# kai422/DAS3R

Measured on AMD Instinct MI355X. Metric: render fwd+bwd Msplats/s at 1080p, higher is better.
Workload: dtype f32; 1 GPU; 1M random splats, 1920x1080, SH degree 3, forward+backward (BASELINE.json configs[3], constant P); splats_per_gpu=1000000, splats_per_gpu_final=1000000, init_steps=30, sh_degree=3, num_rendered=2614506, api=GaussianRasterizer.forward + autograd backward (drop-in surface), parallelism=1 independent scenes, one per GPU

## Files before the change

### das3r_amd/csrc/api.hip

```cpp
#include <stdarg.h>
#include <string.h>

#include <vector>

#include "host_state.h"
#include "preprocess_choice.h"
#include <algorithm>

namespace das3r {

static thread_local char g_err[512] = "";

void set_error(const char *fmt, ...) {
    va_list ap;
    va_start(ap, fmt);
    vsnprintf(g_err, sizeof(g_err), fmt, ap);
    va_end(ap);
}

struct ProfRec {
    const char *name;
    hipEvent_t start, stop;
};
static bool g_prof_on = false;
// ... 163 lines not shown
}

using namespace das3r;

extern "C" int das3r_abi_version(void) { return DAS3R_ABI_VERSION; }
extern "C" void das3r_reload_switches(void) { load_switches(); }
extern "C" void das3r_debug_inject_fault(uint32_t bits) {
    g_inject_fault = (int)bits;
    load_switches();
}
extern "C" void das3r_debug_mutate(uint32_t what) {
    g_mutate = (int)what;
    load_switches();
}
extern "C" const char *das3r_last_error(void) { return g_err; }
extern "C" int das3r_split_colour_switch(void) { return switches().split_colour; }
extern "C" int das3r_split_colour_rule(int32_t has_sh, int32_t sh_degree, int32_t P, int32_t binning_path, int32_t no_backward, int32_t forced) {
    return split_colour_rule(has_sh != 0, sh_degree, P, binning_path, no_backward != 0, forced) ? 1 : 0;
}

namespace {
struct PolicyOnState {
    Verdict v;
    Resume r;
    das3r_path_policy_state *s;
    explicit PolicyOnState(das3r_path_policy_state *state) : s(state) { policy_state_from(*s, &v, &r); }
    ~PolicyOnState() { policy_state_to(v, r, s); }
    PolicyInputs inputs(const das3r_path_policy_inputs *in) {
        return PolicyInputs{in->P, in->W, in->H, in->ntiles, in->tbits, in->tile_passes, in->too_long, in->want_bits, in->forced, in->onesweep != 0,
                            in->capacity_hint, in->capacity_exact != 0, &r};
    }
};
ForwardPlan plan_of(const das3r_path_policy_plan *p) {
    return ForwardPlan{p->local != 0, p->seg != 0, p->seg_bits, p->seg_passes, p->speculate != 0, p->cap, p->decide_fine != 0, p->gen};
}
}
extern "C" void das3r_debug_path_policy_fresh(das3r_path_policy_state *state, uint32_t gen) { policy_state_to(Verdict::fresh(gen), Resume(), state); }
extern "C" void das3r_debug_path_policy_plan(das3r_path_policy_state *state, const das3r_path_policy_inputs *in, das3r_path_policy_plan *out) {
    PolicyOnState on(state);
    const ForwardPlan p = plan_forward(on.v, on.inputs(in));
    *out = das3r_path_policy_plan{p.local, p.seg, p.seg_bits, p.seg_passes, p.speculate, p.decide_fine, p.gen, p.cap};
}
extern "C" int das3r_debug_path_policy_count(das3r_path_policy_state *state, const das3r_path_policy_inputs *in, const das3r_path_policy_plan *plan, int64_t I) {
    PolicyOnState on(state);
    return learn_count(on.v, I, on.inputs(in), plan_of(plan)) ? 1 : 0;
}
extern "C" int das3r_debug_path_policy_skew(das3r_path_policy_state *state, uint32_t longest, uint32_t crowd16, int64_t cap, int32_t ntiles) {
    PolicyOnState on(state);
    return learn_skew(on.v, longest, crowd16, cap, ntiles) ? 1 : 0;
}
extern "C" uint32_t das3r_debug_path_policy_hint(const das3r_path_policy_state *state) {
    Verdict v;
    Resume r;
    policy_state_from(*state, &v, &r);
    return backward_hint(v, (uint32_t)BUCKET);
}
extern "C" void das3r_debug_path_policy_forget(das3r_path_policy_state *state) {
    PolicyOnState on(state);
    forget(on.v);
}
extern "C" void das3r_debug_path_policy_resume(das3r_path_policy_state *state, uint32_t fine, uint32_t forwards) {
    PolicyOnState on(state);
    resume(on.v, on.r, fine != 0u, forwards);
}
extern "C" int das3r_debug_seg_dbits(int32_t tbits, int32_t passes) { return seg_dbits((int)tbits, (int)passes); }

extern "C" void das3r_debug_parse_switches(const char *const *names, const char *const *values, int32_t n, int32_t experiments, das3r_switches *out) {
    auto lookup = [&](const char *name) -> const char * {
        for (int32_t i = 0; i < n; i++)
            if (strcmp(names[i], name) == 0) return values[i];
        return nullptr;
    };
    switches_to(parse_switches(lookup, experiments != 0), out);
}
// ... 415 lines not shown
```

### das3r_amd/csrc/common.h

```cpp
#pragma once
#include <hip/hip_runtime.h>
#include <stdint.h>
#include <stdio.h>

#include "../../include/das3r_raster.h"
#include "kernel_choice.h"
#include "path_policy.h"
#include "pretransform_math.h"

#define TILE_X 16
#define TILE_Y 16
#define TILE_PIX 256
#define WAVE 64
#define NEAR_PLANE 0.001f

namespace das3r {

void set_error(const char *fmt, ...);

const Switches &switches();

#define HIP_TRY(expr)                                                                          \
    do {                                                                                       \
        hipError_t _e = (expr);                                                                \
// ... 112 lines not shown
constexpr uint32_t SHJAC_SAVED_FLAG = 4u;
constexpr uint32_t NO_BACKWARD_IN_FLAG = 8u;
constexpr uint32_t ANTIALIAS_FLAG = 16u;
struct Layout {
    das3r_raster_layout pub;
    size_t g_keyA, g_keyB, g_valA, g_valB, g_hist, g_totals, g_blocksums, g_count, g_off_by_gid, g_rect;
    size_t b_keyA, b_keyB, b_valA, b_valB, b_hist, b_totals, b_gid_of, b_slot;
    size_t b_e2;
    size_t b_ckpt;
    size_t d_ckpt, d_recs, d_dpix, d_bg, d_dz, d_bytes;
    size_t g_ghist, g_ticket, g_status, g_scan_status, g_ctrl_bytes;
    int64_t capacity;
    size_t b_ghist, b_ticket, b_status, b_ctrl_bytes;
    int tiles_x, tiles_y, ntiles, tbits, tile_passes;
    int chunksP, chunksI;
    int dbits, kbits, kshift;
    int part_passes;
    size_t g_dhist;
    size_t g_shjac;
    const uint32_t *dhist_ptr;
    size_t i_order;
};
static inline int seg_dbits(const Layout &L, int passes) { return seg_dbits(L.tbits, passes); }

struct LocalBin {
    float4 *ckpt;
    uint32_t *point_list, *slot_list;
    uint32_t *keys;
    uint32_t *host_flag;
    uint32_t flag_value;
    uint32_t last_g, cap;
    bool prefer_regions;
    const uint32_t *tile_order;
};
void compute_layout(int P, int64_t I, int W, int H, Layout *L, bool shjac = false);

struct EmitArgs {
    unsigned long long *status;
    uint32_t tag;
    uint32_t *ghist;
    uint32_t *err;
    uint32_t *tile_keys, *gids, *off_by_gid;
    uint32_t cap;
    int tbits;
    uint32_t *count;
    uint32_t *count_out;
};
constexpr int EMIT_SLOT_WORDS = 64 + 4 * 256;
constexpr int EMIT_STATUS_GRANULES = 1024;

constexpr int COLOUR_WGS_PER_CU = 4;
struct SideStream {
    hipStream_t stream;
    hipEvent_t fork, join;
    int colour_blocks;
};
int launch_preprocess(const das3r_raster_args *a, const das3r_raster_in *in, int32_t *radii, char *geom, char *img, char *binning_ctrl,
                      size_t binning_ctrl_bytes, const Layout &L, unsigned long long *arrive, uint32_t *host_out, uint32_t tag,
                      hipStream_t s, const EmitArgs *emit, uint32_t *dhist, uint32_t *dhist_next, bool aa ,
                      const SideStream *side = nullptr);
int launch_sh_colour(const das3r_raster_args *a, const das3r_raster_in *in, char *geom, const Layout &L, const SideStream *side);
int launch_mark_visible(int P, const float *means3D, const float *viewmatrix, uint8_t *present, hipStream_t s);
int launch_depth_sort(int P, char *geom, const Layout &L, int part, char *binning_ctrl, size_t binning_ctrl_bytes, bool debug, hipStream_t s);
int launch_scan(int P, char *geom, const Layout &L, uint32_t *host_out, uint32_t tag, bool debug, hipStream_t s, bool index_order = false);
int launch_scan_emit(int P, int64_t cap, const int32_t *radii, char *geom, char *binning, const Layout &L, uint32_t *host_out, uint32_t tag,
                     bool debug, hipStream_t s, bool index_order = false);
// ... 12 lines not shown
        x = PreXform{p->xyz, p->rot, p->scaling, p->opacity_raw, p->conf_flat, p->mask_index, p->R, p->t, p->Lq};
    }
    return x;
}
int launch_render_forward_regions(const das3r_raster_args *a, float *out_color, char *geom, char *binning, char *img, const Layout &L, const LocalBin &lb,
                                  hipStream_t s, float *out_invdepth, float4 *dckpt);
int launch_tile_lpt(char *img, const Layout &L, uint32_t cap, bool debug, hipStream_t s);
int launch_list_skew(const char *img, const char *binning, const char *geom, const Layout &L, uint32_t cap, uint32_t last_g, uint32_t *mailbox_words, uint32_t tag,
                     bool debug, hipStream_t s);
int launch_render_forward_slices(const das3r_raster_args *a, float *out_color, char *geom, char *binning, char *img, const Layout &L, const LocalBin &lb,
                                 hipStream_t s);
int launch_render_forward_lanes(const das3r_raster_args *a, float *out_color, char *geom, char *binning, char *img, const Layout &L,
                                const LocalBin &lb, hipStream_t s, float *out_invdepth, float4 *dckpt);
int launch_render_forward_rows(const das3r_raster_args *a, float *out_color, char *geom, char *binning, char *img, const Layout &L,
                               const LocalBin &lb, hipStream_t s, float *out_invdepth, float4 *dckpt);
int launch_render_backward_mfma(const das3r_raster_args *a, const float *dL_dpix, char *geom, char *binning, char *img, const Layout &L,
                                float *partial, hipStream_t s);
size_t stream_scratch_bytes(int64_t capacity);
int launch_render_backward_stream(const das3r_raster_args *a, const float *dL_dpix, char *geom, char *binning, char *img, const Layout &L,
                                  float *scratch, hipStream_t s);
int launch_render_backward_scan(const das3r_raster_args *a, const float *dL_dpix, char *geom, char *binning, char *img, const Layout &L,
                                float *partial, const BwdChoice &c, hipStream_t s);
int launch_render_backward_blk(const das3r_raster_args *a, const float *dL_dpix, char *geom, char *binning, char *img, const Layout &L,
                               float *partial, const BwdChoice &c, hipStream_t s);
int launch_render_backward_regions(const das3r_raster_args *a, const float *dL_dpix, char *geom, char *binning, char *img, const Layout &L,
                               float *partial, const BwdChoice &c, hipStream_t s);
constexpr int LOCAL_MAX = 1024;
bool grid_is_resident(int nblocks);
bool use_onesweep();
bool use_tight_rect();
int launch_binning(int P, int64_t I, int W, int H, const int32_t *radii, char *geom, char *binning, char *img, const Layout &L,
                   bool fused_scan, uint32_t *host_late, uint32_t tag, bool debug, hipStream_t s, uint32_t **dead_keys = nullptr,
                   uint32_t *emit_slot = nullptr ,
                   uint32_t *seg_host_flag = nullptr, uint32_t seg_flag_value = 0 );
int launch_segment_sort(int64_t cap, const uint32_t *n_ptr, const uint32_t *keys_final, int fbits, uint32_t *point_list, uint32_t *slot_list,
                        const uint32_t *depth_key, uint32_t last_g, uint32_t *scratch_keys, uint32_t *host_flag, uint32_t flag_value, bool debug,
                        hipStream_t s, int dbits, uint2 *ranges, const uint32_t *err, uint32_t *host_late, uint32_t tag, uint32_t inject);
int launch_render_forward(const das3r_raster_args *a, const float *colors_precomp, float *out_color, char *geom, char *binning,
                          char *img, const Layout &L, const LocalBin &lb, hipStream_t s, float *out_invdepth ,
                          float4 *dckpt );
int launch_depth_pass_inputs(int P, int npix, const char *geom, const Layout &L, char *binning, const float *dL_dinvdepth, hipStream_t s, bool debug);
int launch_depth_fold(int P, const char *geom, const Layout &L, float *partial, const float *partial_depth, float *dz, hipStream_t s, bool debug);
size_t focal_workspace_bytes(int P);
int launch_focal_grad(const das3r_raster_args *a, const das3r_raster_in *in, const char *geom, const Layout &L, const float *partial, bool quad_rows,
                      bool aa , float *sums , float *per_splat , float *workspace, hipStream_t s);
static inline const uint8_t *quad_rows_exist(const float *partial, const Layout &L, bool quad_rows) {
    const size_t cap_rows = L.capacity > 0 ? (size_t)L.capacity : 1;
    return quad_rows ? reinterpret_cast<const uint8_t *>(partial) + align_up(cap_rows * 4 * 12 * sizeof(float)) : nullptr;
}
int launch_render_backward(const das3r_raster_args *a, const float *dL_dpix, char *geom, char *binning, char *img, const Layout &L,
                           float *partial, hipStream_t s, bool *quad_rows, int64_t num_rendered, uint32_t fwd_flags );
int launch_render_aux_forward(int P, int W, int H, int C, const float *feat, float *out, const char *geom, const char *binning, const char *img,
                              const Layout &L, int64_t num_rendered, bool debug, hipStream_t s);
int launch_render_aux_adjoint(int P, int W, int H, int C, const float *dL_dout, float *dL_dfeat, int accumulate, float *partial, const char *geom,
                              const char *binning, const char *img, const Layout &L, int64_t num_rendered, bool debug, hipStream_t s);
int launch_aux_gather(int P, int C, const float *partial, float *dL_dfeat, const char *geom, const Layout &L, bool debug, hipStream_t s);
int launch_render_aux_backward(int P, int W, int H, int C, const float *feat, const float *dL_dout, const float *dL_dalpha, float *partial,
                               float *partial_f, const char *geom, const char *binning, const char *img, const Layout &L, bool debug, hipStream_t s);
int launch_count_live_pairs(const das3r_raster_args *a, char *geom, char *binning, char *img, const Layout &L, unsigned long long *out, hipStream_t s);
int launch_preprocess_backward(const das3r_raster_args *a, const das3r_raster_in *in, char *geom, char *binning, const Layout &L,
                               const das3r_raster_grads *g, const float *partial, hipStream_t s, bool quad_rows, const float *dz ,
                               bool aa );

#ifdef __HIPCC__
__device__ __forceinline__ int lane_id() { return __lane_id(); }

template <int CTRL, int ROW_MASK>
// ... 29 lines not shown
```

### das3r_amd/csrc/forward.hip

```cpp
#include <string.h>

#include <algorithm>
#include <vector>

#include "host_state.h"

namespace das3r {

constexpr int SPLIT_MIN_P = 1 << 18;
bool split_colour_rule(bool has_sh, int sh_degree, int P, int binning_path, bool no_backward, int forced) {
    if (!has_sh || sh_degree < 1 || binning_path != 1 || forced < 0 || P <= 0) return false;
    if (forced > 0) return true;
    return sh_degree >= 2 && P >= SPLIT_MIN_P && !no_backward;
}

struct PerStream {
    int dev;
    hipStream_t caller;
    SideStream side = {nullptr, nullptr, nullptr, 0};
    uint32_t *dhist = nullptr;
    uint32_t turn = 0;
};
struct PerStreams {
    std::vector<PerStream> all;
// ... 332 lines not shown

int ForwardCall::look_at_lists(LocalBin *lb) {
    int r;
    const int P = a->P;
    const int64_t cap = L.capacity;
    const bool by_shape = cap > 0 && quad_lanes(switches(), L.ntiles, L.capacity, false);
    if (plan.decide_fine && by_shape) {
        const uint32_t tag = next_tag(mb);
        if ((r = launch_list_skew(saved->img, saved->binning, saved->geom, L, (uint32_t)cap, (uint32_t)(P - 1), mb->dev + MB_LONGEST, tag, a->debug != 0, s))) return r;
        if ((r = mailbox_wait(mb, MB_SKEW_TAG, tag, s))) return r;
        const uint32_t longest = mb->host[MB_LONGEST], crowd16 = mb->host[MB_CROWD16];
        const int64_t mean = skew_mean(T->verdict, cap, L.ntiles);
        const bool now_fine = learn_skew(T->verdict, longest, crowd16, cap, L.ntiles);
        if (switches().verbose) fprintf(stderr, "[das3r] tile lists: longest %lld, mean %lld, %.1f of 64 consecutive entries in one quadrant -> %s kernels\n", (long long)longest,
                                        (long long)mean, crowd16 / 16.0, now_fine ? "2x2-region" : "block");
    }
    const bool fine = prefers_regions(T->verdict);
    lb->prefer_regions = fine;
    lb->tile_order = nullptr;
    if (tile_lpt_wanted(switches(), L.ntiles, L.capacity, false, fine)) {
        if ((r = launch_tile_lpt(saved->img, L, (uint32_t)cap, a->debug != 0, s))) return r;
        lb->tile_order = (const uint32_t *)(saved->img + L.i_order);
    }
    if (fine && by_shape) saved->flags |= backward_hint(T->verdict, (uint32_t)BUCKET);
    return DAS3R_OK;
}

int ForwardCall::bin_and_render(bool local_order, bool ctrl_zeroed, uint32_t *count_out, uint32_t count_out_tag, uint32_t *emit_slot) {
    int r;
    const int P = a->P;
    const int64_t cap = L.capacity;
    const bool fused_scan = use_onesweep();
    const bool seg = L.dbits > 0;
    if (!emit_slot) {
        if (fused_scan) {
            if ((r = launch_binning_scan_emit(P, cap, out->radii, saved->geom, saved->binning, L, ctrl_zeroed, count_out, count_out_tag, a->debug != 0,
                                              s, local_order || seg))) return r;
        } else if ((r = launch_scan(P, saved->geom, L, nullptr, 0, a->debug != 0, s))) return r;
    }
    uint32_t *host_late = nullptr;
    if (cap > 0 && (r = claim_check_slot(&host_late))) return r;
    uint32_t *dead_keys = nullptr;
    if ((r = launch_binning(P, cap, a->image_width, a->image_height, out->radii, saved->geom, saved->binning, saved->img, L, fused_scan, host_late, late_tag,
                            a->debug != 0, s, &dead_keys, emit_slot, mb->dev + MB_TOO_LONG, plan.gen))) return r;
    if ((r = colour_launch())) return r;
    LocalBin lb = {(float4 *)(saved->binning + L.b_ckpt), nullptr, nullptr, nullptr, nullptr, plan.gen, (uint32_t)(P - 1), (uint32_t)cap};
    if ((r = look_at_lists(&lb))) return r;
    if (local_order && cap > 0) {
        lb.point_list = (uint32_t *)(saved->binning + L.pub.point_list);
        lb.slot_list = (uint32_t *)(saved->binning + L.b_slot);
        lb.keys = dead_keys;
        lb.host_flag = mb->dev + MB_TOO_LONG;
    }
    if ((r = colour_join())) return r;
    return launch_render_forward(a, in->colors_precomp, out->out_color, saved->geom, saved->binning, saved->img, L, lb, s, out->out_invdepth,
                                 depth ? (float4 *)(saved->binning + L.d_ckpt) : nullptr);
}

int ForwardCall::read_count(int64_t *I) {
    const int rc = mailbox_wait(mb, MB_COUNT_TAG, count_tag, s);
    if (rc) return rc;
    if (a->prefiltered && mb->host[MB_FILTERED] == count_tag) {
        set_error("Point is filtered although prefiltered is set. This shouldn't happen!");
        return DAS3R_ERR_INVALID_ARG;
    }
    *I = (int64_t)mb->host[MB_COUNT];
    if (*I > CAPACITY_MAX) { set_error("num_rendered %lld exceeds 2^31", (long long)*I); return DAS3R_ERR_OVERFLOW; }
    return DAS3R_OK;
}

int ForwardCall::flow_fused_emit(int64_t *I) {
    int rc;
    if (!T->emit_ring) HIP_TRY(hipMalloc((void **)&T->emit_ring, ARRIVE_SLOTS * EMIT_SLOT_BYTES));
    if (T->emit.wants_zeroing(count_tag)) {
        HIP_TRY(hipMemsetAsync(T->emit_ring, 0, ARRIVE_SLOTS * EMIT_SLOT_BYTES, s));
        T->emit.zeroed();
    }
    uint32_t *emit_slot = (uint32_t *)(T->emit_ring + (size_t)(count_tag % ARRIVE_SLOTS) * EMIT_SLOT_BYTES);
    const EmitArgs em = {(unsigned long long *)(emit_slot + EMIT_SLOT_WORDS), count_tag, emit_slot + 64, emit_slot,
                         (uint32_t *)(saved->binning + L.b_keyA), (uint32_t *)(saved->binning + L.b_gid_of),
                         (uint32_t *)(saved->geom + L.g_off_by_gid), (uint32_t)L.capacity, L.tbits, (uint32_t *)(saved->geom + L.g_count), mb->dev};
    T->emit.taken_by(count_tag);
    if ((rc = preprocess(2, &em))) return rc;
    if ((rc = bin_and_render(true, true, nullptr, 0, emit_slot))) return rc;
    T->emit.rearmed();
// ... 64 lines not shown
```

### das3r_amd/csrc/kernel_choice.h

```cpp
#pragma once
#include <stdint.h>
#include <stdlib.h>
#include <string.h>

#include <algorithm>

namespace das3r {

enum FwdKernel : int {
    FWD_AUTO = 0,
    FWD_QUAD = 1,
    FWD_ROWS = 2,
    FWD_LANES = 3,
    FWD_SLICES = 4,
    FWD_REGIONS = 5,
};
enum BwdKernel : int {
    BWD_AUTO = 0,
    BWD_DPP = 1,
    BWD_MFMA = 2,
    BWD_SCAN = 3,
    BWD_STREAM = 5,
    BWD_BLK = 6,
    BWD_REGIONS = 7,
// ... 53 lines not shown
    int ablate;
    int tickets;
    int bwd_pad_lds, fwd_pad_lds;
    int bwd_buckets;
    int inject_fault;
    int mutate;
    bool fwd_no_prefetch;
    int split_colour;
    int tile_strip;
};

template <class Lookup>
static inline Switches parse_switches(Lookup &&lookup, bool experiments) {
    Switches w;
    memset(&w, 0, sizeof(w));
    auto env = [&](const char *k) -> const char * { const char *e = lookup(k); return (e && e[0]) ? e : nullptr; };
    auto number_in = [](const char *e, int none) {
        while (*e && (*e < '0' || *e > '9')) e++;
        return *e ? atoi(e) : none;
    };
    const char *e;
    if (experiments) {
        if ((e = env("DAS3R_SORT_IPL"))) { const int v = atoi(e); w.sort_ipl = (v == 4 || v == 8 || v == 16) ? v : 0; }
        w.sort_classic = (e = env("DAS3R_SORT")) && e[0] == 'c';
        w.no_sh_stage = lookup("DAS3R_NO_SH_STAGE") != nullptr;
        if ((e = env("DAS3R_ABLATE"))) { w.ablate_set = true; w.ablate = atoi(e); }
        if ((e = env("DAS3R_BWD_PAD_LDS"))) w.bwd_pad_lds = atoi(e);
        if ((e = env("DAS3R_FWD_PAD_LDS"))) w.fwd_pad_lds = atoi(e);
        if ((e = env("DAS3R_SCAN_ITEMS"))) { const int v = atoi(e); w.scan_items = (v == 1 || v == 2 || v == 4 || v == 8 || v == 16) ? v : 0; }
        w.fwd_no_prefetch = (e = env("DAS3R_FWD_PREFETCH")) && e[0] == '0';
    }
    w.rect_upstream = (e = env("DAS3R_RECT")) && e[0] == 'u';
    w.verbose = env("DAS3R_VERBOSE") != nullptr;
    if ((e = env("DAS3R_BINNING"))) w.binning = e[0] == 'l' ? 1 : (e[0] == 'r' ? -1 : (e[0] == 's' ? (strchr(e, '3') ? 3 : 2) : 0));
    w.capacity_exact = (e = env("DAS3R_CAPACITY")) && e[0] == 'e';
    w.fused_emit_off = (e = env("DAS3R_FUSED_EMIT")) && e[0] == '0';
    if ((e = env("DAS3R_SPLIT_COLOUR"))) w.split_colour = e[0] == '0' ? -1 : (e[0] == '1' ? 1 : 0);
    w.tile_lpt_off = (e = env("DAS3R_TILE_LPT")) && e[0] == '0';
    if ((e = env("DAS3R_RENDER")))
        w.render_fwd = e[0] == 'q' ? FWD_QUAD : (e[0] == 'r' ? FWD_ROWS : (e[0] == 'l' ? FWD_LANES : (e[0] == 's' ? FWD_SLICES : (e[0] == 'f' ? FWD_REGIONS : FWD_AUTO))));
    if ((e = env("DAS3R_RENDER_BWD"))) {
        w.render_bwd = e[0] == 'd' ? BWD_DPP
                     : e[0] == 'm' ? BWD_MFMA
                     : strncmp(e, "stream", 6) == 0 ? BWD_STREAM
                     : e[0] == 's' ? BWD_SCAN
                     : e[0] == 'b' ? BWD_BLK
                     : e[0] == 'f' ? BWD_REGIONS : BWD_AUTO;
        if (w.render_bwd == BWD_BLK) {
            w.render_bwd_mb = number_in(e, 128);
            const char *pp = strchr(e, 'p');
            w.render_bwd_pix = pp ? atoi(pp + 1) : 0;
            const char *po = strchr(e, 'o');
            w.render_bwd_occ = po ? atoi(po + 1) : 5;
        }
        if (w.render_bwd == BWD_REGIONS) {
            w.render_bwd_mb = number_in(e, 128);
            w.render_bwd_strips = strchr(e, 'q') ? STRIPS_QUADRANT : (strchr(e, 's') ? STRIPS_INTERLEAVED : STRIPS_NONE);
        }
        if (w.render_bwd == BWD_SCAN) {
            w.render_bwd_mb = number_in(e, 256);
            w.render_bwd_atomic = strncmp(e, "scana", 5) == 0 || w.render_bwd_mb >= 1000;
        }
    }
    if ((e = env("DAS3R_BWD_REDUCE"))) { w.bwd_reduce_set = true; w.bwd_reduce_shfl = e[0] == 's'; }
    w.tickets = -1;
    if ((e = env("DAS3R_TICKETS"))) w.tickets = e[0] == 'a' ? 0 : (e[0] == 'n' ? 1 << 30 : ((e[0] >= '1' && e[0] <= '9') ? atoi(e) : -1));
    w.deterministic = (e = env("DAS3R_DETERMINISTIC")) && e[0] != '0';
// ... 114 lines not shown
```

### das3r_amd/csrc/path_policy.h

```cpp
#pragma once
#include <stdint.h>

#include <algorithm>

namespace das3r {

constexpr int64_t LOCAL_AVG = 384;
constexpr int64_t SEG_AVG = 384;
constexpr uint32_t CROWDED16 = 23u * 16u;
constexpr uint32_t FINE_PERIOD = 512;
constexpr int BACKOFF_MIN = 64, BACKOFF_MAX = 4096;
constexpr uint32_t CLEAN_RESET = 256;
constexpr int64_t CAPACITY_MAX = 0x7FFFFF00;

static inline int seg_dbits(int tbits, int passes) { return 8 * (passes < 3 ? passes : 3) - tbits; }

static inline uint32_t next_gen(uint32_t gen) { return gen + 1u ? gen + 1u : 1u; }

struct Verdict {
    int P = 0, W = 0, H = 0;
    int64_t last_I = -1;
    int64_t peak_I = 0;
    int radix_left = 0;
    int backoff = BACKOFF_MIN;
    uint32_t gen = 0;
    int seg_extra = 0;
    bool last_seg = false;
    bool fine = false;
    uint32_t forwards = 0;
    uint32_t clean = 0;
    uint32_t longest = 0;
    static Verdict fresh(uint32_t gen) {
        Verdict v;
        v.gen = gen;
        return v;
    }
};

struct Resume {
    bool valid = false, fine = false;
    uint32_t forwards = 0;
};

struct PolicyInputs {
    int P, W, H;
    int ntiles, tbits, tile_passes;
    uint32_t too_long;
    uint32_t want_bits;
    int forced;
    bool onesweep;
    int64_t capacity_hint;
    bool capacity_exact;
    Resume *resume;
};

struct ForwardPlan {
    bool local, seg;
    int seg_bits, seg_passes;
    bool speculate;
    int64_t cap;
    bool decide_fine;
    uint32_t gen;
};

static inline ForwardPlan plan_forward(Verdict &v, const PolicyInputs &in) {
    if (v.P != in.P || v.W != in.W || v.H != in.H) {
        v = Verdict::fresh(next_gen(v.gen));
        v.P = in.P;
        v.W = in.W;
        v.H = in.H;
        if (in.resume && in.resume->valid) {
            v.fine = in.resume->fine;
            v.forwards = in.resume->forwards;
            in.resume->valid = false;
        }
    }
    ForwardPlan p;
    p.decide_fine = (v.forwards++ & (FINE_PERIOD - 1u)) == 0u;
    if (v.last_I < 0) {
    } else if (in.too_long == v.gen && !(v.last_seg && v.seg_extra == 0 && in.tile_passes < 3 && seg_dbits(in.tbits, in.tile_passes + 1) > 0)) {
        if (v.clean >= CLEAN_RESET) v.backoff = BACKOFF_MIN;
        v.radix_left = v.backoff;
        if (v.backoff < BACKOFF_MAX) v.backoff *= 2;
        v.clean = 0;
        v.gen = next_gen(v.gen);
    } else if (in.too_long == v.gen || in.want_bits == v.gen) {
        v.seg_extra = 1;
        v.gen = next_gen(v.gen);
    }
    const int forced = in.forced;
    p.local = in.onesweep && (forced == 1 || (forced == 0 && v.radix_left == 0 && v.last_I <= LOCAL_AVG * in.ntiles));
    p.seg_passes = in.tile_passes + ((forced == 3 || (forced == 0 && v.seg_extra)) ? 1 : 0);
    p.seg_bits = (in.onesweep && p.seg_passes <= 3) ? seg_dbits(in.tbits, p.seg_passes) : 0;
    p.seg = !p.local && p.seg_bits > 0 && (forced >= 2 || (forced == 0 && v.radix_left == 0 && v.last_I >= 0 &&
                                                            (v.last_I >> std::min(p.seg_bits, 20)) <= SEG_AVG * in.ntiles));
    v.last_seg = p.seg;
    if (p.local || p.seg) v.clean++;
    if (forced == 0 && v.radix_left > 0) v.radix_left--;
    p.speculate = (p.local || p.seg) && v.last_I >= 0 && in.capacity_hint != -1 && !in.capacity_exact;
    p.cap = p.speculate ? std::min(std::max(v.last_I + v.last_I / 4, v.peak_I + v.peak_I / 20) + 4096, CAPACITY_MAX) : 0;
    p.gen = v.gen;
    return p;
}

static inline bool learn_count(Verdict &v, int64_t I, const PolicyInputs &in, const ForwardPlan &p) {
    v.last_I = I;
    v.peak_I = std::max(I, v.peak_I - v.peak_I / 1024);
    return p.local && in.forced == 0 && I > LOCAL_AVG * in.ntiles;
}

static inline int64_t skew_mean(const Verdict &v, int64_t cap, int ntiles) { return (v.last_I > 0 ? v.last_I : cap) / std::max(ntiles, 1); }

static inline bool learn_skew(Verdict &v, uint32_t longest32, uint32_t crowd16, int64_t cap, int ntiles) {
    const int64_t longest = (int64_t)longest32, mean = skew_mean(v, cap, ntiles);
    v.longest = longest32;
    v.fine = (longest > mean + (mean * 4) / 5 && longest >= 4096) || crowd16 >= CROWDED16;
    return v.fine;
}

static inline uint32_t backward_hint(const Verdict &v, uint32_t bucket) { return 1u | (std::min<uint32_t>(63u, v.longest / bucket + 2u) << 8); }

static inline bool prefers_regions(const Verdict &v) { return v.fine; }
static inline uint32_t forwards_seen(const Verdict &v) { return v.forwards; }

static inline void forget(Verdict &v) { v = Verdict::fresh(v.gen); }

static inline void resume(Verdict &v, Resume &r, bool fine, uint32_t forwards) {
    forget(v);
    r.valid = true;
// ... 29 lines not shown
```

### das3r_amd/csrc/render_common.h

```cpp
#pragma once
#include "common.h"

namespace das3r {

struct StagedSplat {
    float4 xyh;
    float4 co;
    float4 rgbd;
};

__device__ __forceinline__ float4 lds_read4(const float4 *p) {
    const float4 v = *p;
    asm volatile("" ::"v"(v.w));
    return v;
}

__device__ __forceinline__ StagedSplat null_splat() {
    StagedSplat z;
    z.xyh = make_float4(0.f, 0.f, -1e30f, -1e30f);
    z.co = make_float4(0.f, 0.f, 0.f, 0.f);
    z.rgbd = make_float4(0.f, 0.f, 0.f, 0.f);
    return z;
}

// ... 202 lines not shown
#pragma unroll
            for (int m = 0; m < H; m++) {
                a[m] = key[lo0 + (m << sh)];
                b[m] = key[hi0 - (m << sh)];
            }
#pragma unroll
            for (int m = 0; m < H; m++) ce64(a[m], b[m]);
#pragma unroll
            for (int t = G - 2; t >= 0; t--)
#pragma unroll
                for (int m = 0; m < H; m++)
                    if (!((m >> t) & 1)) {
                        ce64(a[m], a[m | (1 << t)]);
                        ce64(b[m | (1 << t)], b[m]);
                    }
#pragma unroll
            for (int m = 0; m < H; m++) {
                key[lo0 + (m << sh)] = a[m];
                key[hi0 - (m << sh)] = b[m];
            }
        }
        __builtin_amdgcn_fence(__ATOMIC_ACQ_REL, "wavefront");
        for (int R = lk - G; R > 0;) {
            const int g = R < G ? R : G;
            if (g == 1) butterfly_group<1, E>(key, lane, R);
            else if (g == 2) butterfly_group<2, E>(key, lane, R);
            else if (g == 3) butterfly_group<3, E>(key, lane, R);
            __builtin_amdgcn_fence(__ATOMIC_ACQ_REL, "wavefront");
            R -= g;
        }
    }
}

struct NoMark {
    __device__ __forceinline__ void operator()(int) const {}
};
template <bool DEPTH = false, class Mark = NoMark>
__device__ __forceinline__ bool local_order_tile(const LocalBin &lb, const uint2 range, const float4 *__restrict__ xyh,
                                                 const float4 *__restrict__ conic_opacity, const float4 *__restrict__ rgbd,
                                                 StagedSplat *stage , uint32_t *s_gid , const int tid,
                                                 const Mark mark = Mark()) {
    const int n = (int)(range.y - range.x);
    uint32_t *pl = lb.point_list + range.x, *sl = lb.slot_list + range.x;
    if (n <= TILE_PIX) {
        unsigned long long *s_key = reinterpret_cast<unsigned long long *>(s_gid);
        unsigned long long key = 0;
        uint32_t g = 0, slot = 0;
        float4 r0 = make_float4(0.f, 0.f, 0.f, 0.f), r1 = r0, r2 = r0;
        if (tid < n) {
            g = min(pl[tid], lb.last_g);
            slot = sl[tid];
            r0 = xyh[(size_t)g * SPLAT_REC];
            r1 = conic_opacity[(size_t)g * SPLAT_REC];
            r2 = rgbd[(size_t)g * SPLAT_REC];
            key = ((unsigned long long)__float_as_uint(r2.w) << 32) | (unsigned long long)g;
        }
        if (tid < ((n + 7) & ~7)) s_key[tid] = tid < n ? key : ~0ull;
        __syncthreads();
        if (tid < n) {
            int rank = 0;
            for (int j = 0; j < n; j += 8) {
                unsigned long long o[8];
#pragma unroll
                for (int u = 0; u < 8; u++) o[u] = s_key[j + u];
#pragma unroll
                for (int u = 0; u < 8; u++) rank += o[u] < key ? 1 : 0;
            }
            stage[rank].xyh = r0;
            stage[rank].co = r1;
            if constexpr (DEPTH) stage[rank].rgbd = staged_invz(r2);
            else stage[rank].rgbd = r2;
            pl[rank] = g;
            sl[rank] = slot;
        } else {
            stage[tid] = null_splat();
        }
        return true;
    }
    if (n <= LOCAL_MAX) {
        unsigned long long *s_key = reinterpret_cast<unsigned long long *>(stage);
        uint32_t *s_slot = reinterpret_cast<uint32_t *>(stage) + 2 * LOCAL_MAX;
        const int N = n <= 2 * TILE_PIX ? 2 * TILE_PIX : LOCAL_MAX;
        for (int i = tid; i < N; i += TILE_PIX) {
            unsigned long long k = SORT_PAD;
            if (i < n) {
                const uint32_t g = min(pl[i], lb.last_g);
                s_gid[i] = g;
                s_slot[i] = sl[i];
                k = ((unsigned long long)__float_as_uint(rgbd[(size_t)g * SPLAT_REC].w) << 32) | (unsigned long long)i;
            }
            s_key[i] = k;
        }
        __syncthreads();
        mark(6);
        if (N == 2 * TILE_PIX) {
            if (tid < 64) wave_bitonic_sort<3>(reinterpret_cast<double *>(stage), tid);
        } else {
            bool wide_before = false;
            for (int lk = 1; (1 << (lk - 1)) < n; lk++)
                for (int lj = lk - 1; lj >= 0; lj--) {
                    const bool wide = lj > 6;
                    if (wide || wide_before) __syncthreads();
                    else __builtin_amdgcn_fence(__ATOMIC_ACQ_REL, "wavefront");
                    wide_before = wide;
                    for (int pr = tid; pr < (N >> 1); pr += TILE_PIX) {
                        const int i = ((pr >> lj) << (lj + 1)) | (pr & ((1 << lj) - 1));
                        const int q = (lj == lk - 1) ? (i ^ ((2 << lj) - 1)) : (i | (1 << lj));
                        if (q < n) {
                            const unsigned long long a = s_key[i], b = s_key[q];
                            if (a > b) {
// ... 142 lines not shown
```

### das3r_amd/csrc/sort.hip

```cpp
#include "granule.h"
#include "segkey.h"
#include <algorithm>
#include "splat_math.h"

namespace das3r {

template <int IPL>
__global__ void __launch_bounds__(256) radix_hist_kernel(const uint32_t *__restrict__ keys, uint32_t cap, const uint32_t *__restrict__ n_ptr,
                                                         int shift, uint32_t mask, int nchunks, uint32_t *__restrict__ hist) {
    const uint32_t n = n_ptr ? min(*n_ptr, cap) : cap;
    __shared__ uint32_t cnt[SORT_WAVES_PER_BLOCK][RADIX_SIZE];
    const int lane = __lane_id(), wave = threadIdx.x >> 6;
    const int chunk = blockIdx.x * SORT_WAVES_PER_BLOCK + wave;
    const uint32_t base = (uint32_t)chunk * 64u * (uint32_t)IPL;
    uint32_t k[IPL];
#pragma unroll
    for (int s = 0; s < IPL; s++) {
        const uint32_t i = base + s * 64 + lane;
        k[s] = (chunk < nchunks && i < n) ? keys[i] : 0u;
    }
#pragma unroll
    for (int d = lane; d < RADIX_SIZE; d += 64) cnt[wave][d] = 0;
    __builtin_amdgcn_wave_barrier();
    if (chunk >= nchunks) return;
// ... 220 lines not shown
            prev = t;
        }
    }
}

int launch_depth_sort(int P, char *geom, const Layout &L, int part, char *binning_ctrl, size_t binning_ctrl_bytes, bool debug, hipStream_t s) {
    uint32_t *keyA = (uint32_t *)(geom + L.g_keyA), *keyB = (uint32_t *)(geom + L.g_keyB);
    uint32_t *valA = (uint32_t *)(geom + L.g_valA), *valB = (uint32_t *)(geom + L.g_valB);
    uint32_t *hist = (uint32_t *)(geom + L.g_hist), *totals = (uint32_t *)(geom + L.g_totals);
    if (P == 0) return DAS3R_OK;
    int rc;
    if (use_onesweep()) return launch_onesweep_depth_sort(P, geom, L, part, (uint32_t *)binning_ctrl, (uint32_t)(binning_ctrl_bytes / 4), debug, s);
#ifdef DAS3R_EXPERIMENTS
    if (part == 1) return DAS3R_OK;
    if ((rc = radix_pass(keyA, nullptr, keyB, valB, P, 0, 8, hist, totals, debug, s))) return rc;
    if ((rc = radix_pass(keyB, valB, keyA, valA, P, 8, 8, hist, totals, debug, s))) return rc;
    if ((rc = radix_pass(keyA, valA, keyB, valB, P, 16, 8, hist, totals, debug, s))) return rc;
    if ((rc = radix_pass(keyB, valB, nullptr, valA, P, 24, 8, hist, totals, debug, s))) return rc;
#else
    (void)keyA; (void)keyB; (void)valA; (void)valB; (void)hist; (void)totals; (void)rc;
#endif
    return DAS3R_OK;
}

int launch_binning_scan_emit(int P, int64_t I, const int32_t *radii, char *geom, char *binning, const Layout &L, bool ctrl_zeroed,
                             uint32_t *host_out, uint32_t tag, bool debug, hipStream_t s, bool index_order) {
    if (I == 0 || P == 0) return DAS3R_OK;
    if (!ctrl_zeroed) HIP_TRY(hipMemsetAsync(binning + L.b_ghist, 0, L.b_ctrl_bytes, s));
    return launch_scan_emit(P, I, radii, geom, binning, L, host_out, tag, debug, s, index_order);
}

int launch_binning(int P, int64_t I, int W, int H, const int32_t *radii, char *geom, char *binning, char *img, const Layout &L,
                   bool fused_scan, uint32_t *host_late, uint32_t tag, bool debug, hipStream_t s, uint32_t **dead_keys, uint32_t *emit_slot,
                   uint32_t *seg_host_flag, uint32_t seg_flag_value) {
    const uint32_t *n_ptr = (const uint32_t *)(geom + L.g_count);
    (void)W; (void)H;
    uint2 *ranges = (uint2 *)(img + L.pub.ranges);
    if (I == 0 || P == 0) return DAS3R_OK;
    uint32_t *keyA = (uint32_t *)(binning + L.b_keyA), *keyB = (uint32_t *)(binning + L.b_keyB);
    uint32_t *valA = (uint32_t *)(binning + L.b_valA), *valB = (uint32_t *)(binning + L.b_valB);
    uint32_t *hist = (uint32_t *)(binning + L.b_hist), *totals = (uint32_t *)(binning + L.b_totals);
    uint32_t *gid_of = (uint32_t *)(binning + L.b_gid_of), *inv = (uint32_t *)(binning + L.b_slot);
    const bool onesweep = use_onesweep();
    (void)onesweep;
#ifdef DAS3R_EXPERIMENTS
    if (!fused_scan) {
    const int emit_blocks = div_up(P, 256) < 1024 ? div_up(P, 256) : 1024;
    DAS3R_LAUNCH(emit_kernel, dim3(emit_blocks), dim3(256), 0, s, P, L.tiles_x, L.tiles_y,
                 (const uint32_t *)(geom + L.pub.sorted_idx), (const uint32_t *)(geom + L.pub.tiles_touched),
                 (const uint32_t *)(geom + L.pub.offsets), (const float4 *)(geom + L.pub.xy), radii, keyA, gid_of, (uint32_t)I,
                 onesweep ? (uint32_t *)(binning + L.b_ghist) : (uint32_t *)nullptr, L.tbits, use_tight_rect() ? 1 : 0);
    KERNEL_CHECK(s, debug, "emit");
    }
#else
    (void)radii; (void)fused_scan; (void)gid_of;
#endif
    if (onesweep) {
        uint32_t *kfinal = nullptr;
        int rc1 = launch_onesweep_partition(I, geom, binning, L, &kfinal, debug, s, emit_slot ? emit_slot + 64 : nullptr, emit_slot);
        if (rc1) return rc1;
        if (dead_keys) *dead_keys = kfinal;
        if (L.dbits > 0) {
            uint32_t *other = kfinal == keyA ? keyB : keyA;
            return launch_segment_sort(I, n_ptr, kfinal, L.kshift, (uint32_t *)(binning + L.pub.point_list), (uint32_t *)(binning + L.b_slot),
                                       (const uint32_t *)(geom + L.pub.depth_key), (uint32_t)(P - 1), other, seg_host_flag, seg_flag_value, debug, s,
                                       L.dbits, ranges, (const uint32_t *)(geom + L.g_ticket) + 8, host_late, tag, (uint32_t)switches().inject_fault);
        }
        const int rearm = emit_slot ? EMIT_SLOT_WORDS : 0;
        DAS3R_LAUNCH(tile_ranges_kernel, dim3(div_up(std::max<int64_t>(div_up(I, 4), rearm), 256)), dim3(256), 0, s, (uint32_t)I, n_ptr, kfinal, ranges,
                     emit_slot ? emit_slot : (uint32_t *)(geom + L.g_ticket) + 8, host_late, tag, (uint32_t)rearm, (uint32_t)switches().inject_fault, L.dbits + L.kshift);
        KERNEL_CHECK(s, debug, "tile_ranges");
        return DAS3R_OK;
    }
#ifdef DAS3R_EXPERIMENTS
    uint32_t *kin = keyA, *vin = nullptr, *kout = keyB, *vout = valB;
    int shift = 0, rc;
    for (int p = 0; p < L.tile_passes; p++) {
        const int dw = tile_digit_width(L.tbits), bits = (L.tbits - shift) < dw ? (L.tbits - shift) : dw;
        const bool last = p == L.tile_passes - 1;
        if ((rc = radix_pass(kin, vin, kout, vout, I, shift, bits, hist, totals, debug, s, last ? gid_of : nullptr, last ? inv : nullptr, n_ptr)))
            return rc;
        shift += bits;
        uint32_t *t = kin; kin = kout; kout = t;
        vin = vout;
        vout = (vout == valB) ? valA : valB;
    }
    if (dead_keys) *dead_keys = kin;
    DAS3R_LAUNCH(tile_ranges_kernel, dim3(div_up(div_up(I, 4), 256)), dim3(256), 0, s, (uint32_t)I, n_ptr, kin, ranges,
                 (uint32_t *)(geom + L.g_ticket) + 8, host_late, tag, 0u, (uint32_t)switches().inject_fault, 0);
    KERNEL_CHECK(s, debug, "tile_ranges");
#else
    (void)keyA; (void)keyB; (void)valA; (void)valB; (void)hist; (void)totals; (void)inv;
#endif
    return DAS3R_OK;
}
// ... 3 lines not shown
```

Measured before the change: 1192 Msplats/s.

## Finish coarse depth-bucket sort locally in render tiles instead of segment sort

```diff
diff --git a/das3r_amd/csrc/api.hip b/das3r_amd/csrc/api.hip
--- a/das3r_amd/csrc/api.hip
+++ b/das3r_amd/csrc/api.hip
@@ -219,14 +219,14 @@
     }
 };
 ForwardPlan plan_of(const das3r_path_policy_plan *p) {
-    return ForwardPlan{p->local != 0, p->seg != 0, p->seg_bits, p->seg_passes, p->speculate != 0, p->cap, p->decide_fine != 0, p->gen};
+    return ForwardPlan{p->local != 0, p->seg != 0, p->seg == 2, p->seg_bits, p->seg_passes, p->speculate != 0, p->cap, p->decide_fine != 0, p->gen};
 }
 }
 extern "C" void das3r_debug_path_policy_fresh(das3r_path_policy_state *state, uint32_t gen) { policy_state_to(Verdict::fresh(gen), Resume(), state); }
 extern "C" void das3r_debug_path_policy_plan(das3r_path_policy_state *state, const das3r_path_policy_inputs *in, das3r_path_policy_plan *out) {
     PolicyOnState on(state);
     const ForwardPlan p = plan_forward(on.v, on.inputs(in));
-    *out = das3r_path_policy_plan{p.local, p.seg, p.seg_bits, p.seg_passes, p.speculate, p.decide_fine, p.gen, p.cap};
+    *out = das3r_path_policy_plan{p.local, p.bucket_local ? 2 : (p.seg ? 1 : 0), p.seg_bits, p.seg_passes, p.speculate, p.decide_fine, p.gen, p.cap};
 }
 extern "C" int das3r_debug_path_policy_count(das3r_path_policy_state *state, const das3r_path_policy_inputs *in, const das3r_path_policy_plan *plan, int64_t I) {
     PolicyOnState on(state);
diff --git a/das3r_amd/csrc/common.h b/das3r_amd/csrc/common.h
--- a/das3r_amd/csrc/common.h
+++ b/das3r_amd/csrc/common.h
@@ -168,6 +168,7 @@
     uint32_t last_g, cap;
     bool prefer_regions;
     const uint32_t *tile_order;
+    int dbits, fbits;
 };
 void compute_layout(int P, int64_t I, int W, int H, Layout *L, bool shjac = false);
 
@@ -246,7 +247,8 @@
 int launch_binning(int P, int64_t I, int W, int H, const int32_t *radii, char *geom, char *binning, char *img, const Layout &L,
                    bool fused_scan, uint32_t *host_late, uint32_t tag, bool debug, hipStream_t s, uint32_t **dead_keys = nullptr,
                    uint32_t *emit_slot = nullptr ,
-                   uint32_t *seg_host_flag = nullptr, uint32_t seg_flag_value = 0 );
+                   uint32_t *seg_host_flag = nullptr, uint32_t seg_flag_value = 0 ,
+                   bool local_finish = false );
 int launch_segment_sort(int64_t cap, const uint32_t *n_ptr, const uint32_t *keys_final, int fbits, uint32_t *point_list, uint32_t *slot_list,
                         const uint32_t *depth_key, uint32_t last_g, uint32_t *scratch_keys, uint32_t *host_flag, uint32_t flag_value, bool debug,
                         hipStream_t s, int dbits, uint2 *ranges, const uint32_t *err, uint32_t *host_late, uint32_t tag, uint32_t inject);
diff --git a/das3r_amd/csrc/forward.hip b/das3r_amd/csrc/forward.hip
--- a/das3r_amd/csrc/forward.hip
+++ b/das3r_amd/csrc/forward.hip
@@ -388,6 +388,7 @@
     const int64_t cap = L.capacity;
     const bool fused_scan = use_onesweep();
     const bool seg = L.dbits > 0;
+    const bool finish = seg && plan.bucket_local;
     if (!emit_slot) {
         if (fused_scan) {
             if ((r = launch_binning_scan_emit(P, cap, out->radii, saved->geom, saved->binning, L, ctrl_zeroed, count_out, count_out_tag, a->debug != 0,
@@ -398,15 +399,16 @@
     if (cap > 0 && (r = claim_check_slot(&host_late))) return r;
     uint32_t *dead_keys = nullptr;
     if ((r = launch_binning(P, cap, a->image_width, a->image_height, out->radii, saved->geom, saved->binning, saved->img, L, fused_scan, host_late, late_tag,
-                            a->debug != 0, s, &dead_keys, emit_slot, mb->dev + MB_TOO_LONG, plan.gen))) return r;
+                            a->debug != 0, s, &dead_keys, emit_slot, mb->dev + MB_TOO_LONG, plan.gen, finish))) return r;
     if ((r = colour_launch())) return r;
     LocalBin lb = {(float4 *)(saved->binning + L.b_ckpt), nullptr, nullptr, nullptr, nullptr, plan.gen, (uint32_t)(P - 1), (uint32_t)cap};
     if ((r = look_at_lists(&lb))) return r;
-    if (local_order && cap > 0) {
+    if ((local_order || finish) && cap > 0) {
         lb.point_list = (uint32_t *)(saved->binning + L.pub.point_list);
         lb.slot_list = (uint32_t *)(saved->binning + L.b_slot);
         lb.keys = dead_keys;
         lb.host_flag = mb->dev + MB_TOO_LONG;
+        if (finish) lb.dbits = L.dbits, lb.fbits = L.kshift;
     }
     if ((r = colour_join())) return r;
     return launch_render_forward(a, in->colors_precomp, out->out_color, saved->geom, saved->binning, saved->img, L, lb, s, out->out_invdepth,
diff --git a/das3r_amd/csrc/kernel_choice.h b/das3r_amd/csrc/kernel_choice.h
--- a/das3r_amd/csrc/kernel_choice.h
+++ b/das3r_amd/csrc/kernel_choice.h
@@ -109,7 +109,7 @@
     }
     w.rect_upstream = (e = env("DAS3R_RECT")) && e[0] == 'u';
     w.verbose = env("DAS3R_VERBOSE") != nullptr;
-    if ((e = env("DAS3R_BINNING"))) w.binning = e[0] == 'l' ? 1 : (e[0] == 'r' ? -1 : (e[0] == 's' ? (strchr(e, '3') ? 3 : 2) : 0));
+    if ((e = env("DAS3R_BINNING"))) w.binning = e[0] == 'l' ? 1 : (e[0] == 'r' ? -1 : (e[0] == 's' ? (strchr(e, '3') ? 3 : 2) : (e[0] == 'b' ? 4 : 0)));
     w.capacity_exact = (e = env("DAS3R_CAPACITY")) && e[0] == 'e';
     w.fused_emit_off = (e = env("DAS3R_FUSED_EMIT")) && e[0] == '0';
     if ((e = env("DAS3R_SPLIT_COLOUR"))) w.split_colour = e[0] == '0' ? -1 : (e[0] == '1' ? 1 : 0);
diff --git a/das3r_amd/csrc/path_policy.h b/das3r_amd/csrc/path_policy.h
--- a/das3r_amd/csrc/path_policy.h
+++ b/das3r_amd/csrc/path_policy.h
@@ -7,6 +7,9 @@
 
 constexpr int64_t LOCAL_AVG = 384;
 constexpr int64_t SEG_AVG = 384;
+constexpr int64_t BUCKET_LOCAL_AVG = 256;
+constexpr int BUCKET_LOCAL_TILES = 1024;
+constexpr int BUCKET_LOCAL_DBITS = 2;
 constexpr uint32_t CROWDED16 = 23u * 16u;
 constexpr uint32_t FINE_PERIOD = 512;
 constexpr int BACKOFF_MIN = 64, BACKOFF_MAX = 4096;
@@ -16,6 +19,12 @@
 static inline int seg_dbits(int tbits, int passes) { return 8 * (passes < 3 ? passes : 3) - tbits; }
 
 static inline uint32_t next_gen(uint32_t gen) { return gen + 1u ? gen + 1u : 1u; }
+
+static inline bool bucket_local_rule(int forced, bool onesweep, int tbits, int tile_passes, int ntiles, int64_t last_I, int radix_left) {
+    if (!onesweep || seg_dbits(tbits, tile_passes) < BUCKET_LOCAL_DBITS) return false;
+    if (forced == 4) return true;
+    return forced == 0 && radix_left == 0 && ntiles > BUCKET_LOCAL_TILES && last_I > BUCKET_LOCAL_AVG * ntiles && last_I <= LOCAL_AVG * ntiles;
+}
 
 struct Verdict {
     int P = 0, W = 0, H = 0;
@@ -56,6 +65,7 @@
 
 struct ForwardPlan {
     bool local, seg;
+    bool bucket_local;
     int seg_bits, seg_passes;
     bool speculate;
     int64_t cap;
@@ -89,12 +99,13 @@
         v.gen = next_gen(v.gen);
     }
     const int forced = in.forced;
-    p.local = in.onesweep && (forced == 1 || (forced == 0 && v.radix_left == 0 && v.last_I <= LOCAL_AVG * in.ntiles));
-    p.seg_passes = in.tile_passes + ((forced == 3 || (forced == 0 && v.seg_extra)) ? 1 : 0);
+    p.bucket_local = bucket_local_rule(forced, in.onesweep, in.tbits, in.tile_passes, in.ntiles, v.last_I, v.radix_left);
+    p.local = !p.bucket_local && in.onesweep && (forced == 1 || forced == 4 || (forced == 0 && v.radix_left == 0 && v.last_I <= LOCAL_AVG * in.ntiles));
+    p.seg_passes = in.tile_passes + ((!p.bucket_local && (forced == 3 || (forced == 0 && v.seg_extra))) ? 1 : 0);
     p.seg_bits = (in.onesweep && p.seg_passes <= 3) ? seg_dbits(in.tbits, p.seg_passes) : 0;
-    p.seg = !p.local && p.seg_bits > 0 && (forced >= 2 || (forced == 0 && v.radix_left == 0 && v.last_I >= 0 &&
-                                                            (v.last_I >> std::min(p.seg_bits, 20)) <= SEG_AVG * in.ntiles));
-    v.last_seg = p.seg;
+    p.seg = p.bucket_local || (!p.local && p.seg_bits > 0 && (forced == 2 || forced == 3 || (forced == 0 && v.radix_left == 0 && v.last_I >= 0 &&
+                                                                                              (v.last_I >> std::min(p.seg_bits, 20)) <= SEG_AVG * in.ntiles)));
+    v.last_seg = p.seg && !p.bucket_local;
     if (p.local || p.seg) v.clean++;
     if (forced == 0 && v.radix_left > 0) v.radix_left--;
     p.speculate = (p.local || p.seg) && v.last_I >= 0 && in.capacity_hint != -1 && !in.capacity_exact;
diff --git a/das3r_amd/csrc/render_common.h b/das3r_amd/csrc/render_common.h
--- a/das3r_amd/csrc/render_common.h
+++ b/das3r_amd/csrc/render_common.h
@@ -258,6 +258,10 @@
     }
 }
 
+__device__ __forceinline__ void rank_below(uint32_t &rank, const uint32_t kj, const uint32_t ki) {
+    uint32_t tmp;
+    asm("v_sub_co_u32 %1, vcc, %2, %3\n\tv_addc_co_u32 %0, vcc, 0, %0, vcc" : "+v"(rank), "=&v"(tmp) : "v"(kj), "v"(ki) : "vcc");
+}
 struct NoMark {
     __device__ __forceinline__ void operator()(int) const {}
 };
@@ -302,6 +306,96 @@
             stage[tid] = null_splat();
         }
         return true;
+    }
+    if (lb.dbits > 0 && n <= 2 * TILE_PIX) {
+        uint32_t *s_word = reinterpret_cast<uint32_t *>(stage), *s_byrank = s_word + 2 * TILE_PIX + 8, *s_depth = s_byrank + 2 * TILE_PIX + 8;
+        uint32_t *s_lo = s_depth + 2 * TILE_PIX, *s_hi = s_lo + 128;
+        const uint32_t *kk = lb.keys + range.x;
+        const int wsh = lb.fbits + 9;
+        const uint32_t kmask = (1u << (lb.dbits + lb.fbits)) - 1u;
+        uint32_t g[2], slot[2], w[2], rank[2];
+#pragma unroll
+        for (int u = 0; u < 2; u++) {
+            const int i = u * TILE_PIX + tid;
+            g[u] = slot[u] = 0u;
+            rank[u] = 0xFFFFFFFFu;
+            w[u] = 0xFFFFFFFFu;
+            if (i < n) {
+                g[u] = min(pl[i], lb.last_g);
+                slot[u] = sl[i];
+                w[u] = ((kk[i] & kmask) << 9) | (uint32_t)i;
+            }
+            s_word[i] = w[u];
+        }
+        if (tid < 8) s_word[2 * TILE_PIX + tid] = 0xFFFFFFFFu;
+        __syncthreads();
+#pragma unroll
+        for (int u = 0; u < 2; u++) {
+            const int i = u * TILE_PIX + tid;
+            if (i < n) {
+                const uint32_t b = w[u] >> wsh, before = i ? s_word[i - 1] >> wsh : 0xFFFFFFFFu;
+                if (before != b) {
+                    s_lo[b] = (uint32_t)i;
+                    if (i) s_hi[before] = (uint32_t)i;
+                }
+                if (i == n - 1) s_hi[b] = (uint32_t)n;
+            }
+        }
+        __syncthreads();
+#pragma unroll
+        for (int u = 0; u < 2; u++) {
+            const int i = u * TILE_PIX + tid;
+            if (i < n) {
+                const uint32_t b = w[u] >> wsh, lo = min(s_lo[b], (uint32_t)n) & ~3u, hi = min(s_hi[b], (uint32_t)n);
+                uint32_t r = lo;
+                for (uint32_t j = lo; j < hi; j += 8u) {
+                    const uint4 o = *reinterpret_cast<const uint4 *>(s_word + j), q = *reinterpret_cast<const uint4 *>(s_word + j + 4u);
+                    rank_below(r, o.x, w[u]);
+                    rank_below(r, o.y, w[u]);
+                    rank_below(r, o.z, w[u]);
+                    rank_below(r, o.w, w[u]);
+                    rank_below(r, q.x, w[u]);
+                    rank_below(r, q.y, w[u]);
+                    rank_below(r, q.z, w[u]);
+                    rank_below(r, q.w, w[u]);
+                }
+                rank[u] = min(r, (uint32_t)(n - 1));
+                s_byrank[rank[u]] = w[u];
+            }
+        }
+        __syncthreads();
+        bool tied[2];
+#pragma unroll
+        for (int u = 0; u < 2; u++) {
+            const uint32_t r = rank[u], f = w[u] >> 9;
+            tied[u] = r != 0xFFFFFFFFu && ((r > 0u && (s_byrank[r - 1u] >> 9) == f) || (r + 1u < (uint32_t)n && (s_byrank[r + 1u] >> 9) == f));
+            if (tied[u]) s_depth[r] = __float_as_uint(rgbd[(size_t)g[u] * SPLAT_REC].w);
+        }
+        __syncthreads();
+#pragma unroll
+        for (int u = 0; u < 2; u++)
+            if (tied[u]) {
+                const uint32_t r = rank[u], f = w[u] >> 9, mine = s_depth[r], at = w[u] & 0x1FFu;
+                uint32_t a = r, b = r + 1u, below = 0u;
+                while (a > 0u && (s_byrank[a - 1u] >> 9) == f) a--;
+                while (b < (uint32_t)n && (s_byrank[b] >> 9) == f) b++;
+                for (uint32_t k = a; k < b; k++) {
+                    const uint32_t dk = s_depth[k], pk = s_byrank[k] & 0x1FFu;
+                    below += (dk < mine || (dk == mine && pk < at)) ? 1u : 0u;
+                }
+                rank[u] = a + below;
+            }
+#pragma unroll
+        for (int u = 0; u < 2; u++)
+            if (rank[u] != 0xFFFFFFFFu) s_gid[rank[u]] = g[u];
+        __syncthreads();
+#pragma unroll
+        for (int u = 0; u < 2; u++)
+            if (rank[u] != 0xFFFFFFFFu) {
+                pl[rank[u]] = g[u];
+                sl[rank[u]] = slot[u];
+            }
+        return false;
     }
     if (n <= LOCAL_MAX) {
         unsigned long long *s_key = reinterpret_cast<unsigned long long *>(stage);
diff --git a/das3r_amd/csrc/sort.hip b/das3r_amd/csrc/sort.hip
--- a/das3r_amd/csrc/sort.hip
+++ b/das3r_amd/csrc/sort.hip
@@ -276,7 +276,7 @@
 
 int launch_binning(int P, int64_t I, int W, int H, const int32_t *radii, char *geom, char *binning, char *img, const Layout &L,
                    bool fused_scan, uint32_t *host_late, uint32_t tag, bool debug, hipStream_t s, uint32_t **dead_keys, uint32_t *emit_slot,
-                   uint32_t *seg_host_flag, uint32_t seg_flag_value) {
+                   uint32_t *seg_host_flag, uint32_t seg_flag_value, bool local_finish) {
     const uint32_t *n_ptr = (const uint32_t *)(geom + L.g_count);
     (void)W; (void)H;
     uint2 *ranges = (uint2 *)(img + L.pub.ranges);
@@ -304,7 +304,7 @@
         int rc1 = launch_onesweep_partition(I, geom, binning, L, &kfinal, debug, s, emit_slot ? emit_slot + 64 : nullptr, emit_slot);
         if (rc1) return rc1;
         if (dead_keys) *dead_keys = kfinal;
-        if (L.dbits > 0) {
+        if (L.dbits > 0 && !local_finish) {
             uint32_t *other = kfinal == keyA ? keyB : keyA;
             return launch_segment_sort(I, n_ptr, kfinal, L.kshift, (uint32_t *)(binning + L.pub.point_list), (uint32_t *)(binning + L.b_slot),
                                        (const uint32_t *)(geom + L.pub.depth_key), (uint32_t)(P - 1), other, seg_host_flag, seg_flag_value, debug, s,
```

After: 1208 Msplats/s, median of 6. 1.01x the previous value.
